# Martinsos/edlib

Measured on AMD Instinct MI355X. Metric: GCUPS (cell updates/s), 1M x 150bp HW reads vs 5Mb target, higher is better.
Workload: dtype u32

## Files before the change

edlib_amd/csrc/engine.hpp:

```cpp
#pragma once
#include "../../include/edlib_amd.h"
#include "common.hpp"
#include "pair_kernels.hpp"
#include "lanepair.hpp"
#include "reads_kernels.hpp"
#include "cross_kernels.hpp"
#include "window_kernels.hpp"
#include "strands.hpp"
#include "flat_pairs_prepare.hpp"
#include "pairs_gather.hpp"

#include <chrono>
#include <deque>
#include <functional>
#include <memory>
#include <vector>

namespace edlib_amd {

struct Tables {
    uint8_t tlut[256];
    uint8_t idToByte[256];
    int sigmaT = 0;
    uint32_t presence[8];
// ... 204 lines not shown
        DevBuf<uint32_t> d_peq;
        bool zeroCopy = false; PinBuf hostOut;
        std::vector<int> ovfSlots; std::vector<long long> ovfOff; DevBuf<int> d_ovfPool;
        DevBuf<int> d_lvMap, d_lvBest, d_lvCnt, d_lvPos; std::vector<int> lvMap; int lvS = 0, lvCap = 0; bool lvValid = false;
        DevBuf<int> d_list;
        int nreal = -1;
        bool mates = false; DevBuf<int> d_win;
    };
    static constexpr int kLastLevelCap = 16;
    int listOpenSlots(ReadGroup& g, int kDone, std::vector<int>& out);
    DevBuf<uint8_t> d_selTmp_;
    std::vector<std::unique_ptr<ReadGroup>> groups_;
    DevBuf<uint32_t> d_tpk_, d_trows_;
    DevBuf<unsigned long long> d_wordSteps_;
    PinBuf h_wordSteps_; bool wordStepsPending_ = false;
    DevBuf<unsigned long long> d_ringSteps_; PinBuf h_ringSteps_; bool ringStepsUsed_ = false;
    unsigned long long* ringStepsCounter();
    bool banded_ = false;
    int syms_ = 4;
    int packTarget();
    int runReads();
    int makeGroup(const std::vector<int>& units, int words, std::unique_ptr<ReadGroup>& g, long long oneRoundWaves = 0);
    int runGroupScans(ReadGroup& g, bool fullOnly);
    int runGroupExact(ReadGroup& g);
    int collectGroup(ReadGroup& g, std::vector<UnitResult>& res);
    int seedThreshold(const ReadGroup& g, bool fullOnly) const;
    int buildSeedIndex();
    int runSeedPass(ReadGroup& g, int k);
    DevBuf<uint32_t> d_seedCnt_, d_seedOff_, d_seedPos_;
    DevBuf<uint8_t> d_seedTmp_;
    bool hits_ = false, hitsHaveRun_ = false;
    HitListBuffers hitList_;
    HitRows hostHits_;
    DevBuf<int> d_hitSlotUnit_;
    DevBuf<long long> d_hitTotal_;
    int runReadHits();
    int scanGroupHits(ReadGroup& g, int slotBase);
    int hitsScanBanded(ReadGroup& g, int slotBase, const int* d_slotmap, int nlanes, int numSegments, int segLen, int warm);
    struct Piece { long long off; int len; int thr; };
    int scanPieces(const std::vector<Piece>& pieces, bool filter, std::vector<std::pair<int, int>>* cand,
                   std::vector<uint8_t>* overflow, std::vector<int>* best);
    int solveLongReads(std::vector<UnitResult>& res, std::vector<int>& fallback);
    bool filterScan_ = false;
    struct ChainArgs { const uint32_t* in = nullptr; uint32_t* out = nullptr; const int* src = nullptr; int inLanes = 0, blocks = 0; const int* rowBase = nullptr; };
    ChainArgs chain_;
    int solveTallFull(const std::vector<int>& units, std::vector<UnitResult>& res, std::vector<int>& handBack);
    int collectReads(std::vector<UnitResult>& res);
    bool readsCollected_ = true;
    int scanGroup(ReadGroup& g, int mode, const int* d_slotmap, int nlanes, int kcap, const int* d_kinit,
                  int numSegments, int segLen, int warm, int* segBest, int* segCnt, int* segPos, int cap,
                  const long long* posOff, const int* posCap, bool unbanded = false,
                  unsigned long long* wordSteps = nullptr, const uint32_t* peqDense = nullptr,
                  const int* qlenDense = nullptr, int peqBottom = 0, int* liveBest = nullptr,
                  const Segment* segTable = nullptr, long long tableCols = 0);

    DevBuf<PairDesc> d_descs_;
    DevBuf<unsigned long long> d_peq64_;
    DevBuf<StoreEntry> d_store_;
    DevBuf<int> d_aux_, d_out3_, d_outScore_, d_outCount_, d_outLast_, d_posPool_, d_opsLen_, d_alpha_;
    DevBuf<uint8_t> d_ops_;
    DevBuf<long long> d_opsOff_;
    int solve(int mode, bool wantPositions, bool wantPath, const std::vector<UnitSpec>& units, SolveOut& out,
              int ring = 0, int ringH = 1);
    int solveChunk(int mode, bool wantPositions, bool wantPath, const std::vector<UnitSpec>& units,
                   size_t a, size_t b, SolveOut& out, int ring, int ringH);
    static const int kWide = -1;
    static const int kRing32 = -2;
    bool ring32_fits(const std::vector<UnitSpec>& units, size_t a, size_t b, int G) const;
    DevBuf<unsigned long long> d_wide_; DevBuf<unsigned> d_wabort_; PinBuf h_wabort_;
    int wideCap_ = -1;
    struct WidePlan { int slots = 1; size_t perLaunch = 1; };
    int planWide(int mode, PairDesc* descs, size_t n, WidePlan& plan);
    int launchWide(int mode, const PairScanArgs& a, const PairDesc* hostDescs, size_t n, const WidePlan& plan);
    int checkWide();
    bool wideSerial_ = false;
    bool wideGateHeld_ = false;
    void wideGateRelease();
    int solveWideSplit(const std::vector<UnitSpec>& units, std::vector<int>& out, int ring = 0);
    struct KnownSplit { long long qoff; int m; long long toff; int T; int score; int row, left, right; };
    std::vector<KnownSplit> knownSplits_;
    int solveGlobalDistances(const std::vector<UnitSpec>& units, std::vector<int>& score, std::vector<OpsOut>* paths = nullptr);
    int solveSemiGlobal(int mode, bool wantPositions, const std::vector<UnitSpec>& units, SolveOut& out);
    int solveSemiGlobalUnits(int mode, bool wantPositions, const std::vector<UnitSpec>& units, SolveOut& out);
    int solveBanded(const BandLadder& ladder, bool wantPositions, const std::vector<UnitSpec>& units, SolveOut& out);
    int alphabetLengthsBegin(hipEvent_t after = nullptr);
    bool alphaDeferred_ = false;
    int alphabetLengthsEnd(std::vector<UnitResult>& res);
    std::vector<int> alphaUnits_; bool alphaOnHost_ = false, alphaPending_ = false; long long alphaBytes_ = 0;
    hipStream_t side_ = nullptr;
    DevBuf<int> d_alphaIdx_, d_alphaOut_; PinBuf alphaPin_;
    struct PathPiece { long long qoff; int m; long long toff; int T; int score; };
    int hirschbergLevel(const std::vector<PathPiece>& big, std::vector<int>& splitRow,
                        std::vector<int>& leftScore, std::vector<int>& rightScore);
    int solvePaths(const std::vector<PathPiece>& jobs, std::vector<OpsOut>& opsOut, std::vector<int>& status);
    std::vector<std::shared_ptr<PinBuf>> opsKeep_;
    std::deque<std::vector<uint8_t>> opsOwned_;

    int qlen(int u) const { return (int)(qoff_[u + 1] - qoff_[u]); }
    long long tbase(int u) const { return shared_ ? toff_[0] : toff_[u]; }
    int tlen(int u) const { return shared_ ? (int)(toff_[1] - toff_[0]) : (int)(toff_[u + 1] - toff_[u]); }

    void scanTimerStart();
    void scanTimerStop();
    std::vector<std::pair<hipEvent_t, hipEvent_t>> scanEvents_;
    size_t scanEventsUsed_ = 0;

    std::vector<UnitResult> results_, work_;
// ... 151 lines not shown
```

edlib_amd/csrc/engine_reads.hip:

```cpp
#include "engine.hpp"

#include <algorithm>
#include <chrono>
#include <cmath>
#include <condition_variable>
#include <cstring>
#include <mutex>
#include <thread>

namespace edlib_amd {

__global__ void __launch_bounds__(256)
seed_thresholds_kernel(int* __restrict__ kinit, const int* __restrict__ best, const int* __restrict__ cnt, int n)
{
    const int i = blockIdx.x * blockDim.x + threadIdx.x;
    if (i < n && cnt[i] > 0 && best[i] < kinit[i]) kinit[i] = best[i];
}


int Batch::scanGroup(ReadGroup& g, int mode, const int* d_slotmap, int nlanes, int kcap, const int* d_kinit,
                     int numSegments, int segLen, int warm, int* segBest, int* segCnt, int* segPos, int cap,
                     const long long* posOff, const int* posCap, bool unbanded, unsigned long long* wordSteps,
                     const uint32_t* peqDense, const int* qlenDense, int peqBottom, int* liveBest,
                     const Segment* segTable, long long tableCols)
{
    ReadScanArgs a{};
    a.peq = peqDense ? peqDense : g.d_peq.p; a.tpk = d_tpk_.p; a.trows = d_trows_.p; a.targetLength = tlen(0);
    if (mode == EDLIB_MODE_SHW) a.targetLength = (int)std::min<long long>(a.targetLength, 64LL * g.nwords + 1);
    a.qlen = qlenDense ? qlenDense : g.d_qlen.p; a.kinit = d_kinit; a.slotmap = d_slotmap; a.nlanes = nlanes;
    a.numSegments = numSegments; a.segLen = segLen; a.warm = warm;
    a.segBest = segBest; a.segCnt = segCnt; a.segPos = segPos; a.cap = cap;
    a.posOff = posOff; a.posCap = posCap;
    a.kcap = kcap; a.wordSteps = wordSteps ? wordSteps : d_wordSteps_.p;
    a.filter = filterScan_ ? 1 : 0;
    a.liveBest = liveBest;
    a.segTable = segTable;
    a.bottomAligned = peqBottom;
    a.chainIn = chain_.in; a.chainOut = chain_.out; a.chainSrc = chain_.src; a.chainInLanes = chain_.inLanes;
    a.chainBlocks = chain_.blocks; a.rowBase = chain_.rowBase;
    const bool chained = chain_.in != nullptr || chain_.out != nullptr;
    const bool longGroup = g.nwords > kMaxReadWords;
    const bool fullHeight = banded_ && mode == EDLIB_MODE_HW && unbanded && (chained || syms_ > 4 || longGroup);
    const bool bandedKernel = !fullHeight && banded_ && mode == EDLIB_MODE_HW && (!unbanded || syms_ > 4 || longGroup);
    static const bool dbg = getenv("EDLIB_AMD_DEBUG") != nullptr;
    if (dbg) {
        EDLIB_AMD_HIP(hipStreamSynchronize(stream_));
        fprintf(stderr, "[edlib_amd] scanGroup nwords=%d mode=%d nlanes=%d S=%d segLen=%d warm=%d cap=%d kcap=%d slotmap=%p posOff=%p rows=%s kernel=%s syms=%d\n",
                g.nwords, mode, nlanes, numSegments, segLen, warm, cap, kcap, (const void*)d_slotmap, (const void*)posOff,
                peqBottom > 1 ? "delay" : (peqBottom ? "bottom" : "top"),
                fullHeight ? "full" : (bandedKernel ? "banded" : "plain"), syms_);
        if (peqBottom > 1) fprintf(stderr, "[edlib_amd] scanGroup delayRows=%d\n", peqBottom - 1);
    }
    scanTimerStart();
    const long long colsScanned = segTable ? tableCols
        : std::min<long long>(a.targetLength, (long long)numSegments * segLen) + (long long)(numSegments - 1) * warm;
#ifdef EDLIB_AMD_DRAIN_DIAG
    const char* drainOut = (peqBottom && liveBest) ? "edlib_amd_drain.bin" : nullptr;
    DevBuf<unsigned long long> d_clk;
    const size_t drainGX = ((size_t)(nlanes + 63) / 64 + 3) / 4, drainWaves = drainGX * numSegments * 4;
    if (drainOut) {
        EDLIB_AMD_HIP(d_clk.alloc(2 * drainWaves));
        EDLIB_AMD_HIP(hipMemsetAsync(d_clk.p, 0, 2 * drainWaves * sizeof(unsigned long long), stream_));
        a.waveClock = d_clk.p;
    }
#endif
    if (peqBottom && (fullHeight || bandedKernel)) EDLIB_AMD_HIP(hipErrorInvalidValue);
    if (fullHeight) {
        EDLIB_AMD_HIP(launch_scan_reads_full(g.nwords, syms_, a, stream_));
        stats.word_steps += (long long)((nlanes + 63) / 64 * 64) * g.nwords * colsScanned;
    } else if (bandedKernel) EDLIB_AMD_HIP(launch_scan_reads_banded(g.nwords, syms_, a, stream_));
    else {
        EDLIB_AMD_HIP(launch_scan_reads(g.nwords, mode, a, stream_));
        stats.word_steps += (long long)((nlanes + 63) / 64 * 64) * g.nwords * colsScanned;
    }
    scanTimerStop();
#ifdef EDLIB_AMD_DRAIN_DIAG
    if (drainOut) {
        std::vector<unsigned long long> clk(2 * drainWaves);
        EDLIB_AMD_HIP(hipMemcpyAsync(clk.data(), d_clk.p, clk.size() * sizeof(unsigned long long), hipMemcpyDeviceToHost, stream_));
        EDLIB_AMD_HIP(hipStreamSynchronize(stream_));
        if (FILE* f = fopen(drainOut, "wb")) {
            const unsigned long long head[2] = {drainGX, (unsigned long long)numSegments};
            fwrite(head, sizeof head, 1, f); fwrite(clk.data(), sizeof(unsigned long long), clk.size(), f); fclose(f);
        }
    }
#endif
    if (dbg) {
        EDLIB_AMD_HIP(hipStreamSynchronize(stream_));
        fprintf(stderr, "[edlib_amd] scanGroup done\n");
    }
    return 0;
}

void plan_segments(int nlanes, int T, int mode, int warmFull, long long wantWaves,
                          int& S, int& segLen, int& warm, int minSegCols)
{
    plan_segments_uniform(nlanes, T, mode == EDLIB_MODE_HW, warmFull, wantWaves, minSegCols, S, segLen, warm);
}

int Batch::runReads()
{
    if (groups_.empty()) return 0;
    stats.path |= 1;
    bool seed = false;
// ... 118 lines not shown
            }
        }
    } else {
        if (scanGroup(g, mode, nullptr, g.nslots, twoPass ? kFirst : kNoCap, g.d_kinit.p, g.numSegments, g.segLen,
                      g.warm, g.d_segBest.p, g.d_segCnt.p, g.d_segPos.p, 8, nullptr, nullptr, fullOnly)) return 1;
        const bool chained = chain_.in != nullptr || chain_.out != nullptr;
        EDLIB_AMD_HIP(launch_merge_segments(g.d_segBest.p, g.d_segCnt.p, g.d_segPos.p, g.numSegments, 8,
                                            g.nslots, nullptr, 16, g.d_best.p, g.d_total.p, g.d_pos.p,
                                            g.d_flags.p, stream_, chained ? kOvfRescan : kOvfGatherGroup));
    }
    ladder.push_back(kNoCap);
    int kDone = kFirst;
    for (size_t lv = 0; twoPass && lv < ladder.size(); ++lv) {
        const int kcapL = ladder[lv];
        const bool last = kcapL == kNoCap;
        if (!haveTodo && listOpenSlots(g, kDone, todo)) return 1;
        haveTodo = false;
        if (todo.empty()) break;
        {
            const size_t no = todo.size();
            int S2, segLen2, warm2;
            plan_segments((int)no, T, mode, g.warm, 65536, S2, segLen2, warm2);
            const int capL = last ? kLastLevelCap : 8;
            EDLIB_AMD_HIP(g.d_lvMap.ensure(no));
            int* d_map = g.d_lvMap.p;
            EDLIB_AMD_HIP(hipMemcpyAsync(d_map, todo.data(), no * sizeof(int), hipMemcpyHostToDevice, stream_));
            bool plain = false;
            if (last && no >= 4096) {
                const int np2 = 64;
                std::vector<int> sub(np2);
                for (int i = 0; i < np2; ++i) sub[i] = todo[(size_t)((long long)i * no / np2)];
                int S3, segLen3, warm3;
                plan_segments(np2, T, mode, g.warm, 16384, S3, segLen3, warm3);
                const size_t it3 = (size_t)np2 * S3;
                DevBuf<int> d_m3, d_b3, d_c3, d_p3; DevBuf<unsigned long long> d_ws;
                EDLIB_AMD_HIP(d_m3.alloc(np2)); EDLIB_AMD_HIP(d_b3.alloc(it3)); EDLIB_AMD_HIP(d_c3.alloc(it3));
                EDLIB_AMD_HIP(d_p3.alloc(it3 * 8)); EDLIB_AMD_HIP(d_ws.alloc(1));
                EDLIB_AMD_HIP(hipMemcpyAsync(d_m3.p, sub.data(), np2 * sizeof(int), hipMemcpyHostToDevice, stream_));
                EDLIB_AMD_HIP(hipMemsetAsync(d_ws.p, 0, sizeof(unsigned long long), stream_));
                if (scanGroup(g, mode, d_m3.p, np2, kNoCap, g.d_kinit.p, S3, segLen3, warm3,
                              d_b3.p, d_c3.p, d_p3.p, 8, nullptr, nullptr, false, d_ws.p)) return 1;
                unsigned long long ws = 0;
                EDLIB_AMD_HIP(hipMemcpyAsync(&ws, d_ws.p, sizeof ws, hipMemcpyDeviceToHost, stream_));
                EDLIB_AMD_HIP(hipStreamSynchronize(stream_));
                const double cols = (double)np2 * ((double)T + (double)(S3 - 1) * warm3);
                plain = (double)ws >= 0.85 * g.nwords * cols;
                stats.word_steps += (long long)ws;
            }
            const bool bottomOk = plain && mode == EDLIB_MODE_HW && syms_ == 4 && g.nwords <= kMaxReadWords &&
                                  chain_.in == nullptr && chain_.out == nullptr;
            const int bottom = !bottomOk ? 0 : 1 + delay_rows_for(g.nwords, g.mMax);
            std::vector<Segment> table;
            DevBuf<Segment> d_segTable; long long tableCols = 0;
            if (bottom && S2 > 1 && no >= 4096) {
                int resident = 0;
                EDLIB_AMD_HIP(scan_reads_resident_workgroups(g.nwords, bottom, &resident));
#ifdef EDLIB_AMD_DRAIN_UNIFORM
                resident = 0;
#endif
                table = plan_segments_tapered(T, (int)(((no + 63) / 64 + 3) / 4), resident, warm2, segLen2);
                S2 = (int)table.size();
                for (const Segment& sg : table) tableCols += sg.cols + std::min(warm2, sg.start);
                EDLIB_AMD_HIP(d_segTable.alloc(table.size()));
                EDLIB_AMD_HIP(hipMemcpyAsync(d_segTable.p, table.data(), table.size() * sizeof(Segment), hipMemcpyHostToDevice, stream_));
            }
            const size_t items = no * (size_t)S2;
            EDLIB_AMD_HIP(g.d_lvBest.ensure(items)); EDLIB_AMD_HIP(g.d_lvCnt.ensure(items));
            EDLIB_AMD_HIP(g.d_lvPos.ensure(items * capL));
            int *d_sb = g.d_lvBest.p, *d_sc = g.d_lvCnt.p, *d_sp = g.d_lvPos.p;
            const size_t no64 = (no + 63) / 64 * 64;
            std::vector<int> perm2(no64, -1);
            for (size_t i = 0; i < no; ++i) perm2[i] = g.perm[todo[i]];
            DevBuf<int> d_perm2, d_qlen2, d_kinit2, d_extra2; DevBuf<uint32_t> d_peq2;
            EDLIB_AMD_HIP(d_perm2.alloc(no64)); EDLIB_AMD_HIP(d_qlen2.alloc(no64)); EDLIB_AMD_HIP(d_kinit2.alloc(no64));
            EDLIB_AMD_HIP(d_extra2.alloc(no64)); EDLIB_AMD_HIP(d_peq2.alloc(no64 * (size_t)syms_ * g.nwords));
            EDLIB_AMD_HIP(hipMemcpyAsync(d_perm2.p, perm2.data(), no64 * sizeof(int), hipMemcpyHostToDevice, stream_));
            EDLIB_AMD_HIP(launch_build_peq_reads(g.nwords, syms_, d_qpool_.p, d_qoff_.p, d_perm2.p, (int)no64,
                                                 d_eqtbl_.p, d_presence_.p, cfg_.k, d_peq2.p, d_qlen2.p,
                                                 d_kinit2.p, d_extra2.p, stream_, bottom));
            const int seedCols = 4096;
            DevBuf<int> d_b0, d_c0, d_p0;
            if (mode == EDLIB_MODE_HW && last && no >= 4096 && S2 > 1 && T >= 16 * seedCols) {
                EDLIB_AMD_HIP(d_b0.alloc(no)); EDLIB_AMD_HIP(d_c0.alloc(no)); EDLIB_AMD_HIP(d_p0.alloc(no * 8));
                if (scanGroup(g, mode, nullptr, (int)no, kcapL, d_kinit2.p, 1, seedCols, 0,
                              d_b0.p, d_c0.p, d_p0.p, 8, nullptr, nullptr, plain, nullptr, d_peq2.p, d_qlen2.p, bottom)) return 1;
                hipLaunchKernelGGL(seed_thresholds_kernel, dim3((unsigned)((no + 255) / 256)), dim3(256), 0, stream_,
                                   d_kinit2.p, d_b0.p, d_c0.p, (int)no);
                EDLIB_AMD_HIP(hipGetLastError());
            }
            DevBuf<int> d_live2;
            if (bottom && S2 > 1) {
                EDLIB_AMD_HIP(d_live2.alloc(no64));
                EDLIB_AMD_HIP(hipMemcpyAsync(d_live2.p, d_kinit2.p, no64 * sizeof(int), hipMemcpyDeviceToDevice, stream_));
            }
            if (scanGroup(g, mode, nullptr, (int)no, kcapL, d_kinit2.p, S2, segLen2, warm2,
                          d_sb, d_sc, d_sp, capL, nullptr, nullptr, plain, nullptr, d_peq2.p, d_qlen2.p, bottom, d_live2.p,
                          d_segTable.p, tableCols)) return 1;
            EDLIB_AMD_HIP(launch_merge_segments(d_sb, d_sc, d_sp, S2, capL, (int)no, d_map, 16,
                                                g.d_best.p, g.d_total.p, g.d_pos.p, g.d_flags.p, stream_,
                                                last ? kOvfGatherLevel : kOvfRescan));
            EDLIB_AMD_HIP(hipStreamSynchronize(stream_));
            if (last) { g.lvValid = true; g.lvS = S2; g.lvCap = capL; g.lvMap.swap(todo); }
            if (dbgLadder) fprintf(stderr, "[edlib_amd] level kcap=%d: %zu slots rescanned (plain=%d)\n", kcapL, no, (int)plain);
        }
        kDone = kcapL;
    }
    return 0;
}

int Batch::listOpenSlots(ReadGroup& g, int kDone, std::vector<int>& out)
{
    size_t tmp = 0;
    EDLIB_AMD_HIP(select_slots_scratch_bytes(g.nslots, &tmp));
    EDLIB_AMD_HIP(d_selTmp_.ensure(tmp));
    EDLIB_AMD_HIP(g.d_list.ensure((size_t)g.nslots + 1));
    int* count = g.d_list.p + g.nslots;
    EDLIB_AMD_HIP(launch_select_open_slots(g.d_perm.p, g.d_total.p, g.d_qlen.p, cfg_.k, kDone, g.nslots, g.d_list.p, count,
                                           d_selTmp_.p, d_selTmp_.bytes(), stream_, g.mates));
    int n = 0;
    EDLIB_AMD_HIP(hipMemcpyAsync(&n, count, sizeof(int), hipMemcpyDeviceToHost, stream_));
    EDLIB_AMD_HIP(hipStreamSynchronize(stream_));
    out.resize((size_t)n);
    if (n > 0) {
        EDLIB_AMD_HIP(hipMemcpyAsync(out.data(), g.d_list.p, (size_t)n * sizeof(int), hipMemcpyDeviceToHost, stream_));
        EDLIB_AMD_HIP(hipStreamSynchronize(stream_));
    }
    return 0;
}


int Batch::seedThreshold(const ReadGroup& g, bool fullOnly) const
{
    const long long T = tlen(0);
    if (fullOnly || !banded_ || cfg_.mode != EDLIB_MODE_HW || syms_ != 4 || cfg_.additionalEqualitiesLength > 0 ||
        g.nwords > kMaxReadWords || chain_.in != nullptr || chain_.out != nullptr)
        return -1;
    if (T < 64LL * 32 * g.nwords || g.nslots < 1024 || (long long)g.nslots * T < (1LL << 30)) return -1;
    int kf = -1;
    for (int k = 16; k >= 0 && kf < 0; --k) {
        const int L = g.mMin / (k + 1);
        if (L >= kSeedQ && (double)(k + 1) * (double)T <= std::ldexp(1.0, 2 * L) / 8.0) kf = k;
    }
    return (kf >= 0 && kf >= std::min(8, cfg_.k >= 0 ? cfg_.k : 8)) ? kf : -1;
}

int Batch::buildSeedIndex()
{
    const int T = tlen(0);
    EDLIB_AMD_HIP(d_seedCnt_.ensure((size_t)kSeedBuckets + 1));
    EDLIB_AMD_HIP(d_seedOff_.ensure((size_t)kSeedBuckets + 1));
    EDLIB_AMD_HIP(d_seedPos_.ensure((size_t)T));
    size_t tmp = 0;
    EDLIB_AMD_HIP(seed_index_scratch_bytes(&tmp));
    EDLIB_AMD_HIP(d_seedTmp_.ensure(tmp));
// ... 346 lines not shown
```

edlib_amd/csrc/reads_kernels.hip:

```cpp
#include "reads_kernels.hpp"
#include "reads_scan.hpp"
#include "reads_column_asm.hpp"

namespace edlib_amd {


__global__ void __launch_bounds__(256)
pack_target_2bit_kernel(const uint8_t* __restrict__ raw, const uint8_t* __restrict__ lut,
                        int T, u32* __restrict__ tpk, int nwords)
{
    __shared__ uint8_t s_lut[256];
    s_lut[threadIdx.x] = lut[threadIdx.x];
    __syncthreads();
    const int w = blockIdx.x * blockDim.x + threadIdx.x;
    if (w >= nwords) return;
    const int base = w * 16;
    u32 out = 0;
    if (base + 16 <= T) {
        const uint4 v = *reinterpret_cast<const uint4*>(raw + base);
        const u32 d[4] = {v.x, v.y, v.z, v.w};
#pragma unroll
        for (int i = 0; i < 16; ++i)
            out |= (u32)(s_lut[(d[i >> 2] >> ((i & 3) * 8)) & 0xFF] & 3) << (2 * i);
    } else {
// ... 129 lines not shown
}

hipError_t launch_build_peq_reads(int nwords, int syms, const uint8_t* reads, const long long* qoff,
                                  const int* perm, int nslots, const uint16_t* eqtbl,
                                  const u32* tpres, int kcfg, u32* peq, int* qlen, int* kinit,
                                  int* alphaExtra, hipStream_t stream, int bottomAlign)
{
    if (nslots == 0) return hipSuccess;
    if (!bottom_align_valid(bottomAlign)) return hipErrorInvalidValue;
    if (syms != 4 && syms != 8 && syms != 16) return hipErrorInvalidValue;
    switch (nwords) {
#define CASE(N) case N: return launch_build_peq_t<N>(reads, qoff, perm, nslots, syms, eqtbl, tpres, kcfg, peq, qlen, kinit, alphaExtra, stream, bottomAlign);
        CASE(1) CASE(2) CASE(3) CASE(4) CASE(5) CASE(6) CASE(7) CASE(8) CASE(10) CASE(12) CASE(14) CASE(16) CASE(24) CASE(32)
#undef CASE
    }
    return hipErrorInvalidValue;
}


#define EDLIB_AMD_DISPATCH_COLUMN(sym)                                                     \
    switch (sym) {                                                                         \
        case 0:  column_step<NWD, MODE, BOTTOM>(E0, Pv, Mv, score, sh, zr0, zr1); asm volatile("; sym0"); break; \
        case 1:  column_step<NWD, MODE, BOTTOM>(E1, Pv, Mv, score, sh, zr0, zr1); asm volatile("; sym1"); break; \
        case 2:  column_step<NWD, MODE, BOTTOM>(E2, Pv, Mv, score, sh, zr0, zr1); asm volatile("; sym2"); break; \
        default: column_step<NWD, MODE, BOTTOM>(E3, Pv, Mv, score, sh, zr0, zr1); asm volatile("; sym3"); break; \
    }

#define EDLIB_AMD_DISPATCH_COLUMN_DELAY(FORM, sym)                                         \
    switch (sym) {                                                                         \
        case 0:  column_step_delay<NWD, FORM, R>(E0, Pv, Mv, score, nph, nmh, zr0, zr1); asm volatile("; sym0"); break; \
        case 1:  column_step_delay<NWD, FORM, R>(E1, Pv, Mv, score, nph, nmh, zr0, zr1); asm volatile("; sym1"); break; \
        case 2:  column_step_delay<NWD, FORM, R>(E2, Pv, Mv, score, nph, nmh, zr0, zr1); asm volatile("; sym2"); break; \
        default: column_step_delay<NWD, FORM, R>(E3, Pv, Mv, score, nph, nmh, zr0, zr1); asm volatile("; sym3"); break; \
    }

#define EDLIB_AMD_TRACK_SCORE(sc, col)                         \
    if ((sc) <= best) {                                        \
        if ((sc) < best) { best = (sc); cnt = 0; }             \
        if (cnt < cap) pos[cnt] = (col);                       \
        ++cnt;                                                 \
    }
#define EDLIB_AMD_TRACK(col) EDLIB_AMD_TRACK_SCORE(score, col)

template <int NWD, int MODE, bool BOTTOM = false, int R = 0>
__global__ void __launch_bounds__(256)
scan_reads_kernel(const ReadScanArgs a)
{
    constexpr bool DELAY = R > 0;
    static_assert(R == 0 || R == kDelayRowsShallow || R == kDelayRowsDeep, "delay rows: none, three or seven");
    static_assert(!DELAY || (BOTTOM && MODE == 2), "delay rows: bottom-aligned HW rows");
    constexpr int kHitGroup = DELAY ? R + 1 : 4;
    static_assert(16 % kHitGroup == 0, "no group straddles a 16-column target word");
    const int lane = threadIdx.x & 63;
    const int rblk = blockIdx.x * 4 + (threadIdx.x >> 6);
    const int seg = blockIdx.y;
    const int idx = rblk * 64 + lane;
    if (rblk * 64 >= a.nlanes) return;
    const bool live = idx < a.nlanes;
    const int slot = live ? (a.slotmap ? a.slotmap[idx] : idx) : 0;
#ifdef EDLIB_AMD_DRAIN_DIAG
    if (BOTTOM && a.waveClock && lane == 0)
        a.waveClock[((size_t)blockIdx.y * gridDim.x + blockIdx.x) * 4 + (threadIdx.x >> 6)] = wall_clock64();
#endif

    u32 E0[NWD], E1[NWD], E2[NWD], E3[NWD], Pv[NWD], Mv[NWD];
    {
        const size_t pb = (size_t)(slot >> 6) * 4 * NWD * 64 + (slot & 63);
#pragma unroll
        for (int d = 0; d < NWD; ++d) {
            E0[d] = a.peq[pb + (size_t)(0 * NWD + d) * 64];
            E1[d] = a.peq[pb + (size_t)(1 * NWD + d) * 64];
            E2[d] = a.peq[pb + (size_t)(2 * NWD + d) * 64];
            E3[d] = a.peq[pb + (size_t)(3 * NWD + d) * 64];
            Pv[d] = ~0u;
            Mv[d] = 0u;
        }
    }
    const int m = a.qlen[slot];
    if constexpr (BOTTOM) {
        const int pad = 32 * NWD - R - m;
#pragma unroll
        for (int d = 0; d < NWD; ++d) {
            const int lo = pad - 32 * d;
            Pv[d] = lo <= 0 ? ~0u : (lo >= 32 ? 0u : ~0u << lo);
        }
    }
    const u32 sh = (u32)(m - 1) & 31u;
    u32 zr0 = 0, zr1 = 0;
    if constexpr (BOTTOM && (NWD == 4 || NWD == 5)) {
        asm volatile("v_mov_b32 %0, 0" : "=v"(zr0));
        asm volatile("v_mov_b32 %0, 0" : "=v"(zr1));
    }
    int score = m;
    int best = a.kinit[slot];
    int cnt = 0;
    const long long item = (long long)idx * a.numSegments + seg;
    const int cap = !live ? 0 : (a.posCap ? a.posCap[item] : a.cap);
    int* pos = a.segPos + (!live ? 0 : (a.posOff ? a.posOff[item] : item * a.cap));
    constexpr int kLiveBlocks = kLivePeriod / 16;
    constexpr int kNoImport = 0x1fffffff;
    int* const livep = BOTTOM ? a.liveBest : nullptr;
    int lidx = idx;
    if constexpr (BOTTOM) asm volatile("" : "+v"(lidx));
#define EDLIB_AMD_LIVE_LOAD() (live ? __hip_atomic_load(livep + lidx, __ATOMIC_RELAXED, __HIP_MEMORY_SCOPE_AGENT) : kNoImport)

    const int T = a.targetLength;
    int c0 = seg * a.segLen, c1 = c0 + a.segLen;
    if (a.segTable) { const Segment sg = a.segTable[seg]; c0 = sg.start; c1 = c0 + sg.cols; }
    if (c1 > T) c1 = T;
    int cw = c0 - a.warm; if (cw < 0) cw = 0;
    cw &= ~15;

    u32 nph = 0, nmh = 0;
    for (int w = cw >> 4; w < (c0 >> 4); ++w) {
        const u32 tw = a.tpk[w];
#pragma unroll
        for (int j = 0; j < 16; ++j) {
            const u32 sym = (tw >> (2 * j)) & 3u;
            if constexpr (!DELAY) {
                EDLIB_AMD_DISPATCH_COLUMN(sym)
            } else if ((j & (kHitGroup - 1)) != kHitGroup - 1) {
                EDLIB_AMD_DISPATCH_COLUMN_DELAY(0, sym)
            } else {
                EDLIB_AMD_DISPATCH_COLUMN_DELAY(1, sym)
            }
        }
    }
    const int wend = c1 >> 4;
    int lim = best + (kHitGroup - 1);
    if constexpr (DELAY) {
        int lim2 = 2 * best + kHitGroup;
        for (int w0 = c0 >> 4; w0 < wend; w0 += kLiveBlocks) {
        if (livep) {
            const int got = EDLIB_AMD_LIVE_LOAD();
            if (2 * got + kHitGroup < lim2) { lim2 = 2 * got + kHitGroup; cnt = 0; }
        }
        const int w1 = w0 + kLiveBlocks < wend ? w0 + kLiveBlocks : wend;
        for (int w = w0; w < w1; ++w) {
            const u32 tw = a.tpk[w];
#pragma unroll
            for (int j = 0; j < 16; j += kHitGroup) {
#pragma unroll
                for (int q = 0; q < kHitGroup - 1; ++q) {
                    const u32 sym = (tw >> (2 * (j + q))) & 3u;
                    EDLIB_AMD_DISPATCH_COLUMN_DELAY(0, sym)
                }
                const int before = score;
                {
                    const u32 sym = (tw >> (2 * (j + kHitGroup - 1))) & 3u;
                    EDLIB_AMD_DISPATCH_COLUMN_DELAY(1, sym)
                }
                if (__builtin_expect(score + before <= lim2, 0)) {
                    int sc[kHitGroup], acc = before, least = 0x7fffffff;
#pragma unroll
                    for (int q = 0; q < kHitGroup; ++q) {
                        acc += (int)((nph >> (kHitGroup - 1 - q)) & 1u) - (int)((nmh >> (kHitGroup - 1 - q)) & 1u);
                        sc[q] = acc;
                        least = acc < least ? acc : least;
                    }
                    best = (lim2 - kHitGroup) >> 1;
                    if (least <= best) {
#pragma unroll
                        for (int q = 0; q < kHitGroup; ++q) { EDLIB_AMD_TRACK_SCORE(sc[q], w * 16 + j + q) }
// ... 5 lines not shown
        }
        }
        lim = ((lim2 - kHitGroup) >> 1) + (kHitGroup - 1);
    }
    for (int w0 = c0 >> 4; !DELAY && w0 < wend; w0 += kLiveBlocks) {
    if (livep) {
        const int got = EDLIB_AMD_LIVE_LOAD();
        if (got + (kHitGroup - 1) < lim) { lim = got + (kHitGroup - 1); cnt = 0; }
    }
    const int w1 = w0 + kLiveBlocks < wend ? w0 + kLiveBlocks : wend;
    for (int w = w0; w < w1; ++w) {
        const u32 tw = a.tpk[w];
#pragma unroll
        for (int j = 0; j < 16; j += kHitGroup) {
            int sc[kHitGroup];
#pragma unroll
            for (int q = 0; q < kHitGroup; ++q) {
                const u32 sym = (tw >> (2 * (j + q))) & 3u;
                EDLIB_AMD_DISPATCH_COLUMN(sym)
                sc[q] = score;
            }
            if (MODE != 0) {
                if (__builtin_expect(score <= lim, 0)) {
                    best = lim - (kHitGroup - 1);
#pragma unroll
                    for (int q = 0; q < kHitGroup; ++q) { EDLIB_AMD_TRACK_SCORE(sc[q], w * 16 + j + q) }
                    if (livep && live && best + (kHitGroup - 1) < lim) atomicMin(livep + lidx, best);
                    lim = best + (kHitGroup - 1);
                }
            }
        }
    }
    }
#undef EDLIB_AMD_LIVE_LOAD
    best = lim - (kHitGroup - 1);
    const int rem = c1 - (wend << 4);
    if (rem > 0) {
        u32 tw = a.tpk[wend];
        for (int j = 0; j < rem; ++j) {
            const u32 sym = tw & 3u;
            tw >>= 2;
            if constexpr (DELAY) { EDLIB_AMD_DISPATCH_COLUMN_DELAY(2, sym) } else { EDLIB_AMD_DISPATCH_COLUMN(sym) }
            if (MODE != 0) { EDLIB_AMD_TRACK(wend * 16 + j) }
        }
    }
    if (live) {
        const size_t o = (size_t)lidx * a.numSegments + seg;
        a.segBest[o] = (MODE == 0) ? score : best;
        a.segCnt[o] = (MODE == 0) ? 1 : cnt;
    }
#ifdef EDLIB_AMD_DRAIN_DIAG
    if (BOTTOM && a.waveClock && __builtin_amdgcn_mbcnt_hi(~0u, __builtin_amdgcn_mbcnt_lo(~0u, 0u)) == 0) {
        const int rb = lidx >> 6;
        a.waveClock[((size_t)gridDim.y + blockIdx.y) * gridDim.x * 4 + rb] = wall_clock64();
    }
#endif
}

template <int NWD>
static hipError_t launch_scan_mode(int mode, const ReadScanArgs& a, hipStream_t stream)
{
    const int nrblk = (a.nlanes + 63) / 64;
    dim3 grid((nrblk + 3) / 4, a.numSegments), block(256);
    switch (mode) {
        case 0: hipLaunchKernelGGL((scan_reads_kernel<NWD, 0>), grid, block, 0, stream, a); break;
        case 1: hipLaunchKernelGGL((scan_reads_kernel<NWD, 1>), grid, block, 0, stream, a); break;
        case 2: if (a.bottomAligned == 1 + kDelayRowsDeep) hipLaunchKernelGGL((scan_reads_kernel<NWD, 2, true, kDelayRowsDeep>), grid, block, 0, stream, a);
                else if (a.bottomAligned == 1 + kDelayRowsShallow) hipLaunchKernelGGL((scan_reads_kernel<NWD, 2, true, kDelayRowsShallow>), grid, block, 0, stream, a);
                else if (a.bottomAligned) hipLaunchKernelGGL((scan_reads_kernel<NWD, 2, true>), grid, block, 0, stream, a);
                else hipLaunchKernelGGL((scan_reads_kernel<NWD, 2>), grid, block, 0, stream, a);
                break;
        default: return hipErrorInvalidValue;
    }
    return hipGetLastError();
}

hipError_t launch_scan_reads(int nwords, int mode, const ReadScanArgs& a, hipStream_t stream)
{
    if (a.nlanes == 0) return hipSuccess;
    if (a.bottomAligned && mode != 2) return hipErrorInvalidValue;
    if (!bottom_align_valid(a.bottomAligned)) return hipErrorInvalidValue;
    switch (nwords) {
#define CASE(N) case N: return launch_scan_mode<N>(mode, a, stream);
        CASE(1) CASE(2) CASE(3) CASE(4) CASE(5) CASE(6) CASE(7) CASE(8)
#undef CASE
    }
    return hipErrorInvalidValue;
}

template <int NWD>
static hipError_t resident_bottom(int bottomAligned, int* perCU)
{
    if (bottomAligned == 1 + kDelayRowsDeep) return hipOccupancyMaxActiveBlocksPerMultiprocessor(perCU, scan_reads_kernel<NWD, 2, true, kDelayRowsDeep>, 256, 0);
    if (bottomAligned == 1 + kDelayRowsShallow) return hipOccupancyMaxActiveBlocksPerMultiprocessor(perCU, scan_reads_kernel<NWD, 2, true, kDelayRowsShallow>, 256, 0);
    return hipOccupancyMaxActiveBlocksPerMultiprocessor(perCU, scan_reads_kernel<NWD, 2, true>, 256, 0);
}

hipError_t scan_reads_resident_workgroups(int nwords, int bottomAligned, int* resident)
{
    int dev = 0, cus = 0, perCU = 0;
    hipError_t e = hipGetDevice(&dev);
    if (e == hipSuccess) e = hipDeviceGetAttribute(&cus, hipDeviceAttributeMultiprocessorCount, dev);
    if (e != hipSuccess) return e;
    switch (nwords) {
#define CASE(N) case N: e = resident_bottom<N>(bottomAligned, &perCU); break;
        CASE(1) CASE(2) CASE(3) CASE(4) CASE(5) CASE(6) CASE(7) CASE(8)
#undef CASE
        default: return hipErrorInvalidValue;
    }
    *resident = perCU * cus;
    return e;
}


hipError_t launch_scan_reads_full_long(int nwords, int syms, const ReadScanArgs& a, hipStream_t stream);
hipError_t launch_scan_reads_banded_long(int nwords, int syms, const ReadScanArgs& a, hipStream_t stream);

template <int S, bool CHAIN>
static hipError_t launch_scan_reads_full_s(int nwords, const ReadScanArgs& a, hipStream_t stream)
{
    dim3 grid((a.nlanes + 63) / 64, a.numSegments), block(64);
    switch (nwords) {
#define CASE(N) case N: EDLIB_AMD_CHECK_STATIC_LDS((scan_reads_full_kernel<N, S, CHAIN>), N * S * 256); \
                        hipLaunchKernelGGL((scan_reads_full_kernel<N, S, CHAIN>), grid, block, 0, stream, a); break;
        CASE(1) CASE(2) CASE(3) CASE(4) CASE(5) CASE(6) CASE(7) CASE(8)
#undef CASE
        default: return hipErrorInvalidValue;
    }
    return hipGetLastError();
}

hipError_t launch_scan_reads_full(int nwords, int syms, const ReadScanArgs& a, hipStream_t stream)
{
    if (a.nlanes == 0) return hipSuccess;
    if (a.segTable) return hipErrorInvalidValue;
    if (nwords > kMaxReadWords) return launch_scan_reads_full_long(nwords, syms, a, stream);
    const bool chain = a.chainIn != nullptr || a.chainOut != nullptr;
    switch (syms) {
        case 4: return chain ? launch_scan_reads_full_s<4, true>(nwords, a, stream) : launch_scan_reads_full_s<4, false>(nwords, a, stream);
        case 8: return chain ? launch_scan_reads_full_s<8, true>(nwords, a, stream) : launch_scan_reads_full_s<8, false>(nwords, a, stream);
        case 16: return chain ? launch_scan_reads_full_s<16, true>(nwords, a, stream) : launch_scan_reads_full_s<16, false>(nwords, a, stream);
    }
    return hipErrorInvalidValue;
}

template <int S>
static hipError_t launch_scan_reads_banded_s(int nwords, const ReadScanArgs& a, hipStream_t stream)
{
    const int nrblk = (a.nlanes + 63) / 64;
    dim3 grid(nrblk, a.numSegments), block(64);
    switch (nwords) {
#define CASE(N) case N: if (a.filter) { EDLIB_AMD_CHECK_STATIC_LDS((scan_reads_banded_kernel<N, S, true>), N * S * 256); \
                                            hipLaunchKernelGGL((scan_reads_banded_kernel<N, S, true>), grid, block, 0, stream, a); } \
                        else { EDLIB_AMD_CHECK_STATIC_LDS((scan_reads_banded_kernel<N, S, false>), N * S * 256); \
                               hipLaunchKernelGGL((scan_reads_banded_kernel<N, S, false>), grid, block, 0, stream, a); } break;
        CASE(1) CASE(2) CASE(3) CASE(4) CASE(5) CASE(6) CASE(7) CASE(8)
#undef CASE
        default: return hipErrorInvalidValue;
// ... 168 lines not shown
```

edlib_amd/csrc/reads_kernels.hpp:

```cpp
#pragma once
#include <hip/hip_runtime.h>
#include <stdint.h>

#include "hit_list.hpp"
#include "segment_plan.hpp"

namespace edlib_amd {

constexpr int kMaxReadWords = 8;
constexpr int kMaxLongReadWords = 16;
constexpr int kMaxLongReadWords4 = 32;
constexpr int kFilterFromWords = 13;
inline int read_group_words(int m) { const int w = (m + 31) / 32; return w <= kMaxReadWords ? w : (w <= 10 ? 10 : (w <= 12 ? 12 : (w <= 14 ? 14 : (w <= 16 ? 16 : (w <= 24 ? 24 : 32))))); }
constexpr int kDelayRowsDeep = 7, kDelayRowsShallow = 3;
constexpr bool delay_rows_fit(int nwords, int longest, int rows) { return nwords <= kMaxReadWords && longest >= 1 && longest + rows <= 32 * nwords; }
constexpr int delay_rows_for(int nwords, int longest)
{
    return delay_rows_fit(nwords, longest, kDelayRowsDeep) ? kDelayRowsDeep : (delay_rows_fit(nwords, longest, kDelayRowsShallow) ? kDelayRowsShallow : 0);
}
constexpr bool bottom_align_valid(int b) { return b == 0 || b == 1 || b == 1 + kDelayRowsShallow || b == 1 + kDelayRowsDeep; }
constexpr int kLanes = 64;


struct ReadScanArgs {
    const uint32_t* peq;
    const uint32_t* tpk;
    const uint32_t* trows;
    int targetLength;
    const int* qlen;
    const int* kinit;
    const int* slotmap;
    int nlanes;
    int numSegments;
    int segLen;
    int warm;
    int* segBest;
    int* segCnt;
    int* segPos;
    int cap;
    const long long* posOff;
    const int* posCap;
    int kcap;
    unsigned long long* wordSteps;
    const uint32_t* chainIn; uint32_t* chainOut;
    const int* chainSrc;
    int chainInLanes;
    int chainBlocks;
    const int* rowBase;
    int filter;
    HitList hits;
    int slotBase;
    int bottomAligned;
    int* liveBest;
    const Segment* segTable;
#ifdef EDLIB_AMD_DRAIN_DIAG
    unsigned long long* waveClock;
#endif
};
constexpr int kLivePeriod = 1024;

hipError_t launch_scan_reads(int nwords, int mode, const ReadScanArgs& a, hipStream_t stream);
hipError_t scan_reads_resident_workgroups(int nwords, int bottomAligned, int* resident);

hipError_t launch_scan_reads_banded(int nwords, int syms, const ReadScanArgs& a, hipStream_t stream);

hipError_t launch_scan_reads_full(int nwords, int syms, const ReadScanArgs& a, hipStream_t stream);

hipError_t launch_pack_target_2bit(const uint8_t* raw, const uint8_t* lut, int targetLength,
                                   uint32_t* tpk, hipStream_t stream);
hipError_t launch_pack_target_rows(const uint8_t* raw, const uint8_t* lut, int targetLength,
                                   uint32_t* trows, int ndwords, hipStream_t stream);

hipError_t launch_build_peq_reads(int nwords, int syms, const uint8_t* reads, const long long* qoff,
                                  const int* perm, int nslots, const uint16_t* eqtbl,
                                  const uint32_t* targetPresence , int kcfg,
                                  uint32_t* peq, int* qlen, int* kinit, int* alphaExtra,
                                  hipStream_t stream, int bottomAlign = 0);

hipError_t launch_collect_candidates(const int* segCnt, const int* segPos, int numSegments, int cap, int nlanes,
                                     int* out, int maxOut, int* counter, int* overflow, hipStream_t stream);

constexpr int kSeedQ = 12;
constexpr int kSeedBuckets = 1 << (2 * kSeedQ);
constexpr int kSeedBucketCap = 64;
constexpr int kSeedMaxDiag = 32;
constexpr int kSeedMaxWindow = 1024;

struct SeedArgs {
    const uint32_t* peq;
    const int* qlen;
    const int* perm;
    const uint32_t* tpk;
    int targetLength;
    const uint32_t* seedOff;
    const uint32_t* seedPos;
    int nslots;
    int k;
    int* best; int* total; int* pos; int* flags;
    int* backSlots; int* backCount;
    unsigned long long* wordSteps;
    HitList hits;
    int slotBase;
};

hipError_t seed_index_scratch_bytes(size_t* bytes);
hipError_t launch_build_seed_index(const uint32_t* tpk, int targetLength, uint32_t* cnt, uint32_t* off, uint32_t* pos,
                                   void* tmp, size_t tmpBytes, hipStream_t stream);
hipError_t launch_seed_verify(int nwords, const SeedArgs& a, hipStream_t stream);

hipError_t launch_merge_segments(const int* segBest, const int* segCnt, const int* segPos,
                                 int numSegments, int cap, int nlanes, const int* slotmap, int capFinal,
                                 int* best, int* total, int* pos, int* flags, hipStream_t stream, int gatherFlag = 1);
constexpr int kOvfRescan = 1, kOvfGatherLevel = 2, kOvfGatherGroup = 4;
hipError_t launch_gather_segments(const int* segBest, const int* segCnt, const int* segPos, int numSegments, int cap, int n,
                                  const int* idx, const long long* off, const int* lim, int* out, hipStream_t stream);
// ... 15 lines not shown
```

edlib_amd/csrc/segment_plan.hpp:

```cpp
#pragma once
#include <algorithm>
#include <vector>

namespace edlib_amd {

struct Segment { int start, cols; };

constexpr int kMaxSegments = 65535;

inline int seg_roundup16(long long x) { return (int)((x + 15) / 16 * 16); }

inline void plan_segments_uniform(int nlanes, int T, bool hw, int warmFull, long long wantWaves, int minSegCols,
                                  int& S, int& segLen, int& warm)
{
    S = 1; segLen = seg_roundup16(T); warm = 0;
    if (!hw) return;
    const long long nrblk = ((long long)nlanes + 63) / 64;
    long long want = (wantWaves + nrblk - 1) / nrblk;
    want = std::max(1LL, std::min<long long>(want, std::min(kMaxSegments, std::max(1, T / minSegCols))));
    if (warmFull > 0) want = std::max(1LL, std::min<long long>(want, std::max<long long>(1, T / (4LL * warmFull))));
    segLen = seg_roundup16((T + want - 1) / want);
    S = (T + segLen - 1) / segLen;
    warm = warmFull;
}

inline std::vector<Segment> uniform_segment_table(int T, int Lmax)
{
    std::vector<Segment> t;
    for (long long c = 0; c < T; c += Lmax) t.push_back({(int)c, (int)std::min<long long>(Lmax, T - c)});
    return t;
}

inline std::vector<Segment> plan_segments_tapered(int T, int gridX, int resident, int warm, int Lmax)
{
    Lmax = std::max(16, Lmax / 16 * 16);
    int minCols = std::max(16, seg_roundup16(4LL * warm));
    minCols = std::max(minCols, seg_roundup16(((long long)T + kMaxSegments - 2) / (kMaxSegments - 1)));
    const long long uniformS = ((long long)T + Lmax - 1) / Lmax;
    if (T <= 0 || gridX <= 0 || resident <= 0 || Lmax <= minCols || uniformS * gridX < 2LL * resident)
        return uniform_segment_table(T, Lmax);
    std::vector<Segment> t;
    long long c = 0;
    while (c < T) {
        const long long rem = T - c;
        long long len = rem * gridX / (2LL * resident) / 16 * 16;
        len = std::max<long long>(minCols, std::min<long long>(Lmax, len));
        if (len > rem) len = rem;
        t.push_back({(int)c, (int)len});
        c += len;
    }
    return t;
}

}
```

Baseline: 3.448 million.

## Bound segment warm-up by seeded threshold and make main-scan workgroup size configurable

The seed-threshold kernel now also reduces the maximum per-lane threshold into a device scalar. The tapered main scan reads that scalar and shortens each segment's warm-up overlap to query rows plus max threshold, which skips redundant warm-up columns. Workgroup size for the main launch can be compiled as one or four waves, with the occupancy query and tapered segment planning adjusted to match. It defaults to one wave per block, which changes scheduling granularity. Stats accounting now adds the warm columns actually walked, read back after the scan.

```diff
diff --git a/edlib_amd/csrc/engine.hpp b/edlib_amd/csrc/engine.hpp
--- a/edlib_amd/csrc/engine.hpp
+++ b/edlib_amd/csrc/engine.hpp
@@ -280,7 +280,9 @@
                   const long long* posOff, const int* posCap, bool unbanded = false,
                   unsigned long long* wordSteps = nullptr, const uint32_t* peqDense = nullptr,
                   const int* qlenDense = nullptr, int peqBottom = 0, int* liveBest = nullptr,
-                  const Segment* segTable = nullptr, long long tableCols = 0);
+                  const Segment* segTable = nullptr, long long tableCols = 0,
+                  const int* warmK = nullptr, int warmRows = 0,
+                  int groupWaves = 0);
 
     DevBuf<PairDesc> d_descs_;
     DevBuf<unsigned long long> d_peq64_;
diff --git a/edlib_amd/csrc/engine_reads.hip b/edlib_amd/csrc/engine_reads.hip
--- a/edlib_amd/csrc/engine_reads.hip
+++ b/edlib_amd/csrc/engine_reads.hip
@@ -10,11 +10,26 @@
 
 namespace edlib_amd {
 
+#ifndef EDLIB_AMD_MAIN_GROUP_WAVES
+#define EDLIB_AMD_MAIN_GROUP_WAVES 1
+#endif
+constexpr int kMainLaunchGroupWaves = EDLIB_AMD_MAIN_GROUP_WAVES;
+static_assert(kMainLaunchGroupWaves == 1 || kMainLaunchGroupWaves == 4, "one wave or four");
+
 __global__ void __launch_bounds__(256)
-seed_thresholds_kernel(int* __restrict__ kinit, const int* __restrict__ best, const int* __restrict__ cnt, int n)
+seed_thresholds_kernel(int* __restrict__ kinit, const int* __restrict__ best, const int* __restrict__ cnt, int n,
+                       int* __restrict__ kmax)
 {
     const int i = blockIdx.x * blockDim.x + threadIdx.x;
-    if (i < n && cnt[i] > 0 && best[i] < kinit[i]) kinit[i] = best[i];
+    int k = 0;
+    if (i < n) {
+        k = kinit[i];
+        if (cnt[i] > 0 && best[i] < k) kinit[i] = k = best[i];
+    }
+    if (kmax) {
+        for (int d = 32; d > 0; d >>= 1) k = max(k, __shfl_xor(k, d, 64));
+        if ((threadIdx.x & 63) == 0) atomicMax(kmax, k);
+    }
 }
 
 
@@ -22,7 +37,7 @@
                      int numSegments, int segLen, int warm, int* segBest, int* segCnt, int* segPos, int cap,
                      const long long* posOff, const int* posCap, bool unbanded, unsigned long long* wordSteps,
                      const uint32_t* peqDense, const int* qlenDense, int peqBottom, int* liveBest,
-                     const Segment* segTable, long long tableCols)
+                     const Segment* segTable, long long tableCols, const int* warmK, int warmRows, int groupWaves)
 {
     ReadScanArgs a{};
     a.peq = peqDense ? peqDense : g.d_peq.p; a.tpk = d_tpk_.p; a.trows = d_trows_.p; a.targetLength = tlen(0);
@@ -35,6 +50,8 @@
     a.filter = filterScan_ ? 1 : 0;
     a.liveBest = liveBest;
     a.segTable = segTable;
+    a.warmK = warmK; a.warmRows = warmRows;
+    a.groupWaves = groupWaves;
     a.bottomAligned = peqBottom;
     a.chainIn = chain_.in; a.chainOut = chain_.out; a.chainSrc = chain_.src; a.chainInLanes = chain_.inLanes;
     a.chainBlocks = chain_.blocks; a.rowBase = chain_.rowBase;
@@ -50,6 +67,12 @@
                 peqBottom > 1 ? "delay" : (peqBottom ? "bottom" : "top"),
                 fullHeight ? "full" : (bandedKernel ? "banded" : "plain"), syms_);
         if (peqBottom > 1) fprintf(stderr, "[edlib_amd] scanGroup delayRows=%d\n", peqBottom - 1);
+        if (groupWaves) fprintf(stderr, "[edlib_amd] scanGroup blockThreads=%d\n", 64 * groupWaves);
+        if (warmK) {
+            int kmax = 0;
+            EDLIB_AMD_HIP(hipMemcpy(&kmax, warmK, sizeof(int), hipMemcpyDeviceToHost));
+            fprintf(stderr, "[edlib_amd] scanGroup warmBound=%d rows=%d kmax=%d\n", warm_bound(warm, warmRows, kmax), warmRows, kmax);
+        }
     }
     scanTimerStart();
     const long long colsScanned = segTable ? tableCols
@@ -274,13 +297,15 @@
             const int bottom = !bottomOk ? 0 : 1 + delay_rows_for(g.nwords, g.mMax);
             std::vector<Segment> table;
             DevBuf<Segment> d_segTable; long long tableCols = 0;
+            int groupWaves = 0;
             if (bottom && S2 > 1 && no >= 4096) {
+                groupWaves = kMainLaunchGroupWaves;
                 int resident = 0;
-                EDLIB_AMD_HIP(scan_reads_resident_workgroups(g.nwords, bottom, &resident));
+                EDLIB_AMD_HIP(scan_reads_resident_workgroups(g.nwords, bottom, groupWaves, &resident));
 #ifdef EDLIB_AMD_DRAIN_UNIFORM
                 resident = 0;
 #endif
-                table = plan_segments_tapered(T, (int)(((no + 63) / 64 + 3) / 4), resident, warm2, segLen2);
+                table = plan_segments_tapered(T, (int)(((no + 63) / 64 + groupWaves - 1) / groupWaves), resident, warm2, segLen2);
                 S2 = (int)table.size();
                 for (const Segment& sg : table) tableCols += sg.cols + std::min(warm2, sg.start);
                 EDLIB_AMD_HIP(d_segTable.alloc(table.size()));
@@ -302,13 +327,23 @@
                                                  d_kinit2.p, d_extra2.p, stream_, bottom));
             const int seedCols = 4096;
             DevBuf<int> d_b0, d_c0, d_p0;
+            DevBuf<int> d_kmax;
+            const bool boundWarm = !table.empty() && g.mMax > 0 && warm2 > 0;
             if (mode == EDLIB_MODE_HW && last && no >= 4096 && S2 > 1 && T >= 16 * seedCols) {
                 EDLIB_AMD_HIP(d_b0.alloc(no)); EDLIB_AMD_HIP(d_c0.alloc(no)); EDLIB_AMD_HIP(d_p0.alloc(no * 8));
+                if (boundWarm) {
+                    EDLIB_AMD_HIP(d_kmax.alloc(1));
+                    EDLIB_AMD_HIP(hipMemsetAsync(d_kmax.p, 0, sizeof(int), stream_));
+                }
                 if (scanGroup(g, mode, nullptr, (int)no, kcapL, d_kinit2.p, 1, seedCols, 0,
                               d_b0.p, d_c0.p, d_p0.p, 8, nullptr, nullptr, plain, nullptr, d_peq2.p, d_qlen2.p, bottom)) return 1;
                 hipLaunchKernelGGL(seed_thresholds_kernel, dim3((unsigned)((no + 255) / 256)), dim3(256), 0, stream_,
-                                   d_kinit2.p, d_b0.p, d_c0.p, (int)no);
+                                   d_kinit2.p, d_b0.p, d_c0.p, (int)no, d_kmax.p);
                 EDLIB_AMD_HIP(hipGetLastError());
+                if (d_kmax.p) {
+                    tableCols = 0;
+                    for (const Segment& sg : table) tableCols += sg.cols;
+                }
             }
             DevBuf<int> d_live2;
             if (bottom && S2 > 1) {
@@ -317,11 +352,21 @@
             }
             if (scanGroup(g, mode, nullptr, (int)no, kcapL, d_kinit2.p, S2, segLen2, warm2,
                           d_sb, d_sc, d_sp, capL, nullptr, nullptr, plain, nullptr, d_peq2.p, d_qlen2.p, bottom, d_live2.p,
-                          d_segTable.p, tableCols)) return 1;
+                          d_segTable.p, tableCols, d_kmax.p, g.mMax - 1, groupWaves)) return 1;
             EDLIB_AMD_HIP(launch_merge_segments(d_sb, d_sc, d_sp, S2, capL, (int)no, d_map, 16,
                                                 g.d_best.p, g.d_total.p, g.d_pos.p, g.d_flags.p, stream_,
                                                 last ? kOvfGatherLevel : kOvfRescan));
+            int kmax = 0;
+            if (d_kmax.p) EDLIB_AMD_HIP(hipMemcpyAsync(&kmax, d_kmax.p, sizeof(int), hipMemcpyDeviceToHost, stream_));
             EDLIB_AMD_HIP(hipStreamSynchronize(stream_));
+            if (d_kmax.p) {
+                const int warmUsed = warm_bound(warm2, g.mMax - 1, kmax);
+                long long warmCols = 0;
+                for (const Segment& sg : table) warmCols += warm_columns_walked(sg.start, warmUsed);
+                stats.word_steps += (long long)no64 * g.nwords * warmCols;
+                if (dbgLadder) fprintf(stderr, "[edlib_amd] level warm-up: %d of %d columns (rows %d + threshold %d), %lld + %lld columns per lane in %d segments\n",
+                                       warmUsed, warm2, g.mMax - 1, kmax, tableCols, warmCols, S2);
+            }
             if (last) { g.lvValid = true; g.lvS = S2; g.lvCap = capL; g.lvMap.swap(todo); }
             if (dbgLadder) fprintf(stderr, "[edlib_amd] level kcap=%d: %zu slots rescanned (plain=%d)\n", kcapL, no, (int)plain);
         }
diff --git a/edlib_amd/csrc/reads_kernels.hip b/edlib_amd/csrc/reads_kernels.hip
--- a/edlib_amd/csrc/reads_kernels.hip
+++ b/edlib_amd/csrc/reads_kernels.hip
@@ -205,7 +205,7 @@
     constexpr int kHitGroup = DELAY ? R + 1 : 4;
     static_assert(16 % kHitGroup == 0, "no group straddles a 16-column target word");
     const int lane = threadIdx.x & 63;
-    const int rblk = blockIdx.x * 4 + (threadIdx.x >> 6);
+    const int rblk = blockIdx.x * (int)(blockDim.x >> 6) + (threadIdx.x >> 6);
     const int seg = blockIdx.y;
     const int idx = rblk * 64 + lane;
     if (rblk * 64 >= a.nlanes) return;
@@ -213,7 +213,7 @@
     const int slot = live ? (a.slotmap ? a.slotmap[idx] : idx) : 0;
 #ifdef EDLIB_AMD_DRAIN_DIAG
     if (BOTTOM && a.waveClock && lane == 0)
-        a.waveClock[((size_t)blockIdx.y * gridDim.x + blockIdx.x) * 4 + (threadIdx.x >> 6)] = wall_clock64();
+        a.waveClock[(size_t)blockIdx.y * ((gridDim.x * (blockDim.x >> 6) + 3) & ~3u) + rblk] = wall_clock64();
 #endif
 
     u32 E0[NWD], E1[NWD], E2[NWD], E3[NWD], Pv[NWD], Mv[NWD];
@@ -261,7 +261,9 @@
     int c0 = seg * a.segLen, c1 = c0 + a.segLen;
     if (a.segTable) { const Segment sg = a.segTable[seg]; c0 = sg.start; c1 = c0 + sg.cols; }
     if (c1 > T) c1 = T;
-    int cw = c0 - a.warm; if (cw < 0) cw = 0;
+    int warm = a.warm;
+    if (a.warmK) { const int need = a.warmRows + *a.warmK; warm = need < warm ? need : warm; }
+    int cw = c0 - warm; if (cw < 0) cw = 0;
     cw &= ~15;
 
     u32 nph = 0, nmh = 0;
@@ -373,7 +375,7 @@
 #ifdef EDLIB_AMD_DRAIN_DIAG
     if (BOTTOM && a.waveClock && __builtin_amdgcn_mbcnt_hi(~0u, __builtin_amdgcn_mbcnt_lo(~0u, 0u)) == 0) {
         const int rb = lidx >> 6;
-        a.waveClock[((size_t)gridDim.y + blockIdx.y) * gridDim.x * 4 + rb] = wall_clock64();
+        a.waveClock[((size_t)gridDim.y + blockIdx.y) * ((gridDim.x * (blockDim.x >> 6) + 3) & ~3u) + rb] = wall_clock64();
     }
 #endif
 }
@@ -382,7 +384,9 @@
 static hipError_t launch_scan_mode(int mode, const ReadScanArgs& a, hipStream_t stream)
 {
     const int nrblk = (a.nlanes + 63) / 64;
-    dim3 grid((nrblk + 3) / 4, a.numSegments), block(256);
+    const int gw = a.groupWaves ? a.groupWaves : 4;
+    if (gw != 1 && gw != 4) return hipErrorInvalidValue;
+    dim3 grid((nrblk + gw - 1) / gw, a.numSegments), block(64 * gw);
     switch (mode) {
         case 0: hipLaunchKernelGGL((scan_reads_kernel<NWD, 0>), grid, block, 0, stream, a); break;
         case 1: hipLaunchKernelGGL((scan_reads_kernel<NWD, 1>), grid, block, 0, stream, a); break;
@@ -410,21 +414,22 @@
 }
 
 template <int NWD>
-static hipError_t resident_bottom(int bottomAligned, int* perCU)
-{
-    if (bottomAligned == 1 + kDelayRowsDeep) return hipOccupancyMaxActiveBlocksPerMultiprocessor(perCU, scan_reads_kernel<NWD, 2, true, kDelayRowsDeep>, 256, 0);
-    if (bottomAligned == 1 + kDelayRowsShallow) return hipOccupancyMaxActiveBlocksPerMultiprocessor(perCU, scan_reads_kernel<NWD, 2, true, kDelayRowsShallow>, 256, 0);
-    return hipOccupancyMaxActiveBlocksPerMultiprocessor(perCU, scan_reads_kernel<NWD, 2, true>, 256, 0);
-}
-
-hipError_t scan_reads_resident_workgroups(int nwords, int bottomAligned, int* resident)
-{
+static hipError_t resident_bottom(int bottomAligned, int threads, int* perCU)
+{
+    if (bottomAligned == 1 + kDelayRowsDeep) return hipOccupancyMaxActiveBlocksPerMultiprocessor(perCU, scan_reads_kernel<NWD, 2, true, kDelayRowsDeep>, threads, 0);
+    if (bottomAligned == 1 + kDelayRowsShallow) return hipOccupancyMaxActiveBlocksPerMultiprocessor(perCU, scan_reads_kernel<NWD, 2, true, kDelayRowsShallow>, threads, 0);
+    return hipOccupancyMaxActiveBlocksPerMultiprocessor(perCU, scan_reads_kernel<NWD, 2, true>, threads, 0);
+}
+
+hipError_t scan_reads_resident_workgroups(int nwords, int bottomAligned, int groupWaves, int* resident)
+{
+    if (groupWaves != 1 && groupWaves != 4) return hipErrorInvalidValue;
     int dev = 0, cus = 0, perCU = 0;
     hipError_t e = hipGetDevice(&dev);
     if (e == hipSuccess) e = hipDeviceGetAttribute(&cus, hipDeviceAttributeMultiprocessorCount, dev);
     if (e != hipSuccess) return e;
     switch (nwords) {
-#define CASE(N) case N: e = resident_bottom<N>(bottomAligned, &perCU); break;
+#define CASE(N) case N: e = resident_bottom<N>(bottomAligned, 64 * groupWaves, &perCU); break;
         CASE(1) CASE(2) CASE(3) CASE(4) CASE(5) CASE(6) CASE(7) CASE(8)
 #undef CASE
         default: return hipErrorInvalidValue;
diff --git a/edlib_amd/csrc/reads_kernels.hpp b/edlib_amd/csrc/reads_kernels.hpp
--- a/edlib_amd/csrc/reads_kernels.hpp
+++ b/edlib_amd/csrc/reads_kernels.hpp
@@ -53,6 +53,9 @@
     int bottomAligned;
     int* liveBest;
     const Segment* segTable;
+    const int* warmK;
+    int warmRows;
+    int groupWaves;
 #ifdef EDLIB_AMD_DRAIN_DIAG
     unsigned long long* waveClock;
 #endif
@@ -60,7 +63,7 @@
 constexpr int kLivePeriod = 1024;
 
 hipError_t launch_scan_reads(int nwords, int mode, const ReadScanArgs& a, hipStream_t stream);
-hipError_t scan_reads_resident_workgroups(int nwords, int bottomAligned, int* resident);
+hipError_t scan_reads_resident_workgroups(int nwords, int bottomAligned, int groupWaves, int* resident);
 
 hipError_t launch_scan_reads_banded(int nwords, int syms, const ReadScanArgs& a, hipStream_t stream);
 
diff --git a/edlib_amd/csrc/segment_plan.hpp b/edlib_amd/csrc/segment_plan.hpp
--- a/edlib_amd/csrc/segment_plan.hpp
+++ b/edlib_amd/csrc/segment_plan.hpp
@@ -23,6 +23,13 @@
     S = (T + segLen - 1) / segLen;
     warm = warmFull;
 }
+
+inline int warm_bound(int warm, int rows, int kmax)
+{
+    return (int)std::max<long long>(0, std::min<long long>(warm, (long long)rows + kmax));
+}
+
+inline int warm_columns_walked(int start, int warm) { return start - (std::max(0, start - warm) & ~15); }
 
 inline std::vector<Segment> uniform_segment_table(int T, int Lmax)
 {
```

After: 3.467 million, median of 6. Within noise of the previous version (+0.6%).
